# Kyaw-Thiha/animal-vision

Hardware: AMD Instinct MI355X
Metric: megapixels/sec per-frame pipeline (higher is better)
Workload: dtype f16

## Files before the change

### animal-vision_amd/csrc/mst_fused.hip

```cpp
#include <hip/hip_fp16.h>

#include <cstdio>
#include <cstdlib>
#include <cstring>

#include "avx_internal.h"
#include "mst_common.h"
#include "mst_tile_order.h"

namespace {

typedef float float4_t __attribute__((ext_vector_type(4)));
#ifndef AVX_FFN32_GM2
#define AVX_FFN32_GM2 1
#endif
constexpr int kFT = 512;
constexpr int TS = 16;
constexpr int HS = TS + 2;
#ifndef AVX_FFN_TH
#define AVX_FFN_TH 16
#endif
constexpr int kFfnTH = AVX_FFN_TH;
static_assert(kFfnTH == 14 || kFfnTH == 16, "FeedForward tile rows");
constexpr int kFfnNGRP = (HS * (kFfnTH + 2) + 31) / 32;
// ... 753 lines not shown
        uint2 xr[STASH ? 1 : NOUT];
        const int yo0 = t.y0 + 2 * rpo + (q >> 1), xo = t.x0 + n16;
        const bool livex = n16 < TW && xo < W;
        const size_t e0 = ((t.b * H + (yo0 < H ? yo0 : 0)) * (size_t)W + (livex ? xo : 0)) * C + 8 * oc + 4 * (q & 1), estep = (size_t)2 * W * C;
        auto live = [&](int u) { return livex && yo0 + 2 * u < H; };
        if constexpr (!STASH) {
#pragma unroll
            for (int u = 0; u < NOUT; ++u) xr[u] = live(u) ? *reinterpret_cast<const uint2*>(x + e0 + u * estep) : uint2{0, 0};
        }
        {
            const bool mid_inside = t.y0 >= 1 && t.y0 + MR - 1 <= H && t.x0 >= 1 && t.x0 + 15 <= W;
            uint4 bq[3];
            auto rd = [&](int u) {
#pragma unroll
                for (int i = 0; i < 3; ++i) bq[i] = *reinterpret_cast<const uint4*>(rbB + (size_t)(2 * (rpo + u)) * RP + i * PP + ob);
            };
            auto finish = [&](int u, float4_t a) {
                float2_t gp[2] = {float2_t{a[0], a[1]}, float2_t{a[2], a[3]}};
                if constexpr (C >= 64) gelu_mx<2>(gp);
                else { float2_t g0[1] = {gp[0]}, g1[1] = {gp[1]}; gelu_mx<1>(g0); gelu_mx<1>(g1); gp[0] = g0[0]; gp[1] = g1[0]; }
                uint2 ov = uint2{pack_f16(gp[0].x, gp[0].y), pack_f16(gp[1].x, gp[1].y)};
                if (!mid_inside) {
                    const int yy = t.y0 - 1 + 2 * (rpo + u) + (q >> 1), xx = t.x0 - 1 + n16;
                    const unsigned keep = (yy >= 0 && yy < H && xx >= 0 && xx < W) ? 0xffffffffu : 0u;
                    ov.x &= keep; ov.y &= keep;
                }
                *reinterpret_cast<uint2*>(wbB + (size_t)(2 * (rpo + u)) * MP + ob) = ov;
            };
            rd(0);
            float4_t prev = {0.f, 0.f, 0.f, 0.f};
#pragma unroll
            for (int u = 0; u < NMID; ++u) {
                float4_t acc = {0.f, 0.f, 0.f, 0.f};
#pragma unroll
                for (int i = 0; i < 3; ++i) acc = __builtin_amdgcn_mfma_f32_16x16x32_f16(a1[i], __builtin_bit_cast(half8_t, bq[i]), acc, 0, 0, 0);
                if (u + 1 < NMID) rd(u + 1);
                __builtin_amdgcn_sched_barrier(0);
                if (u > 0) finish(u - 1, prev);
                __builtin_amdgcn_sched_barrier(0);
                prev = acc;
            }
            finish(NMID - 1, prev);
        }
        stamp(2);
        {
            uint4 bq[3], bg[NK];
            uint2 xn = uint2{0, 0};
            const unsigned char* rbX = xs + (size_t)((q >> 1) * TW + n16) * PP + 16 * o + 8 * (q & 1);
            auto rd = [&](int u) {
#pragma unroll
                for (int i = 0; i < 3; ++i) bq[i] = *reinterpret_cast<const uint4*>(rbC + (size_t)(2 * (rpo + u)) * MP + i * PP + ob);
#pragma unroll
                for (int t2 = 0; t2 < NK; ++t2) bg[t2] = *reinterpret_cast<const uint4*>(rbG + (size_t)(2 * (rpo + u)) * RP + 32 * t2);
                if constexpr (STASH) xn = *reinterpret_cast<const uint2*>(rbX + (size_t)(2 * (rpo + u)) * TW * PP);
            };
            auto finish = [&](int u, float4_t acc, uint2 xu) {
                if (live(u)) {
                    constexpr unsigned kOnes = 0x3c003c00u;
                    float s0 = acc[0] + bs[0], s1 = acc[1] + bs[1], s2 = acc[2] + bs[2], s3 = acc[3] + bs[3];
                    fma_mix_lo(s0, xu.x, kOnes); fma_mix_hi(s1, xu.x, kOnes);
                    fma_mix_lo(s2, xu.y, kOnes); fma_mix_hi(s3, xu.y, kOnes);
                    *reinterpret_cast<uint2*>(out + e0 + u * estep) = uint2{pack_f16(s0, s1), pack_f16(s2, s3)};
                }
            };
            rd(0);
#ifndef AVX_TAIL_PIPE2
#define AVX_TAIL_PIPE2 1
#endif
            if constexpr (STASH && (AVX_TAIL_PIPE2 == 2 || (AVX_TAIL_PIPE2 == 1 && C == 64))) {
                float4_t prev = {0.f, 0.f, 0.f, 0.f};
                uint2 xp = uint2{0, 0};
#pragma unroll
                for (int u = 0; u < NOUT; ++u) {
                    const uint2 xu = xn;
                    float4_t acc = {0.f, 0.f, 0.f, 0.f};
#pragma unroll
                    for (int i = 0; i < 3; ++i) acc = __builtin_amdgcn_mfma_f32_16x16x32_f16(a2[i], __builtin_bit_cast(half8_t, bq[i]), acc, 0, 0, 0);
#pragma unroll
                    for (int t2 = 0; t2 < NK; ++t2) acc = __builtin_amdgcn_mfma_f32_16x16x32_f16(am[t2], __builtin_bit_cast(half8_t, bg[t2]), acc, 0, 0, 0);
                    if (u + 1 < NOUT) rd(u + 1);
                    __builtin_amdgcn_sched_barrier(0);
                    if (u > 0) finish(u - 1, prev, xp);
                    __builtin_amdgcn_sched_barrier(0);
                    prev = acc; xp = xu;
                }
                finish(NOUT - 1, prev, xp);
            } else {
#pragma unroll
                for (int u = 0; u < NOUT; ++u) {
                    const uint2 xu = STASH ? xn : xr[STASH ? 0 : u];
                    float4_t acc = {0.f, 0.f, 0.f, 0.f};
#pragma unroll
                    for (int i = 0; i < 3; ++i) acc = __builtin_amdgcn_mfma_f32_16x16x32_f16(a2[i], __builtin_bit_cast(half8_t, bq[i]), acc, 0, 0, 0);
#pragma unroll
                    for (int t2 = 0; t2 < NK; ++t2) acc = __builtin_amdgcn_mfma_f32_16x16x32_f16(am[t2], __builtin_bit_cast(half8_t, bg[t2]), acc, 0, 0, 0);
                    if (u + 1 < NOUT) rd(u + 1);
                    finish(u, acc, xu);
                }
            }
        }
        }
        stamp(3);
        if (!ahead.live) break;
        t = tile_at(ahead, TW, TR);
        ahead.advance();
        __syncthreads();
        stamp(4);
    }
    if constexpr (STAMP) {
        if (lane == 0 && stamps)
#pragma unroll
            for (int kk = 0; kk < 8; ++kk) stamps[((size_t)blockIdx.x * NW + wave) * 8 + kk] = seg[kk];
    }
}

template <int C, int TR, int MINW, int NW = 8>
int launch_attn_tail_mx(avx_ctx* ctx, const void* x, const void* wvpack, const void* mpack, const void* dw1, const void* dw2, const float* bias, void* out, int B, int H, int W,
                        hipStream_t s) {
    constexpr int PP = C * 2 + 16, RP = (18 * PP + 255) / 256 * 256;
    const size_t lds = (size_t)(TR + 4) * RP + (size_t)(TR + 2) * 16 * PP + (size_t)(C / 32) * (C / 16) * 1024 + ((C <= 64 && NW == 8) ? (size_t)(TR * 14 + 2) * PP : 0) ;
    const long total = (long)B * ((H + TR - 1) / TR) * ((W + 13) / 14);
    const long cap = (long)ctx->num_cus * (NW == 16 ? 1 : MINW / 2);
    AVX_REQUIRE(ctx, total <= 0x7fffffffl, "avx_mst_attn_tail_mx: 2^31 tiles or more");
    const unsigned blocks = (unsigned)(total < cap ? total : cap);
    if (getenv("AVX_TAIL_STAMPS")) {
        auto ks = k_mst_attn_tail_mx<C, TR, MINW, true, NW>;
        unsigned long long* d_st = nullptr;
        const size_t n = (size_t)blocks * NW * 8;
        AVX_HIP(ctx, hipMalloc((void**)&d_st, n * sizeof(unsigned long long)));
        AVX_HIP(ctx, hipFuncSetAttribute((const void*)ks, hipFuncAttributeMaxDynamicSharedMemorySize, (int)lds));
        hipLaunchKernelGGL(ks, dim3(blocks), dim3(64 * NW), lds, s, (const __half*)x, (const uint4*)wvpack, (const uint4*)mpack, (const uint4*)dw1, (const uint4*)dw2, bias, (__half*)out, B, H, W, d_st, mst_tile_order());
        AVX_HIP(ctx, hipStreamSynchronize(s));
        unsigned long long* h_st = (unsigned long long*)malloc(n * sizeof(unsigned long long));
        AVX_HIP(ctx, hipMemcpy(h_st, d_st, n * sizeof(unsigned long long), hipMemcpyDeviceToHost));
        double tot[8] = {0}, all = 0;
        for (size_t i = 0; i < n; ++i) { tot[i & 7] += (double)h_st[i]; all += (double)h_st[i]; }
        const char* nm[8] = {"v from x", "bar1", "conv1+gelu", "conv2+proj+store", "bar2", "-", "-", "-"};
        fprintf(stderr, "[tail stamps C=%d] %u blocks, %ld tiles, mean cycles per wave %.0f:", C, blocks, total, all / (blocks * (double)NW));
        for (int k2 = 0; k2 < 8; ++k2) fprintf(stderr, "  %s %.1f%%", nm[k2], 100 * tot[k2] / all);
        fprintf(stderr, "\n");
        free(h_st);
        (void)hipFree(d_st);
        return AVX_OK;
    }
    auto k = k_mst_attn_tail_mx<C, TR, MINW, false, NW>;
    AVX_HIP(ctx, hipFuncSetAttribute((const void*)k, hipFuncAttributeMaxDynamicSharedMemorySize, (int)lds));
    hipLaunchKernelGGL(k, dim3(blocks), dim3(64 * NW), lds, s, (const __half*)x, (const uint4*)wvpack, (const uint4*)mpack, (const uint4*)dw1,
                       (const uint4*)dw2, bias, (__half*)out, B, H, W, (unsigned long long*)nullptr, mst_tile_order());
    AVX_HIP(ctx, hipGetLastError());
    return AVX_OK;
}


struct SpecStat3 { float mn, mx; double sum; };
template <int MINW, bool GRAM, bool SPEC = false>
__global__ __launch_bounds__(kFT, MINW) void k_mst_conv3x3_lds(const __half* __restrict__ x , const uint4* __restrict__ wpack ,
                                                               const __half* __restrict__ add , __half* __restrict__ out, int B, int H, int W,
                                                               const uint4* __restrict__ wqk , float* __restrict__ partial ,
                                                               const float* __restrict__ specw = nullptr ,
                                                               float* __restrict__ planes = nullptr , SpecStat3* __restrict__ spart = nullptr ,
                                                               int crop_t = 0, int crop_l = 0, int Hc = 0, int Wc = 0, int order = AVX_TILE_ORDER_RASTER ) {
    constexpr int C = 32, PP = C * 2 + 16, RP = (HS * PP + 255) / 256 * 256, NFILL = (HS * HS * 4 + kFT - 1) / kFT;
    __shared__ __align__(16) unsigned char xt[HS * RP];
    __shared__ uint4 wl[18 * 64];
    const int tid = threadIdx.x, lane = tid & 63, wave = tid >> 6, p = lane & 31, h = lane >> 5;
    for (int i = tid; i < 18 * 64; i += kFT) wl[i] = wpack[i];
    __shared__ uint4 wq[GRAM ? 4 * 64 : 1];
    float16_t G;
    float nq = 0.f, nk = 0.f;
    if constexpr (GRAM) {
        if (tid < 4 * 64) wq[tid] = wqk[tid];
#pragma unroll
        for (int v = 0; v < 16; ++v) G[v] = 0.f;
    }
    float smn[3] = {3.4e38f, 3.4e38f, 3.4e38f}, smx[3] = {-3.4e38f, -3.4e38f, -3.4e38f};
    double ssum[3] = {0.0, 0.0, 0.0};
    const int tx = (W + TS - 1) / TS, ty = (H + TS - 1) / TS;
    uint4 pre[NFILL];
    unsigned f_rel[NFILL];
#pragma unroll
    for (int k = 0; k < NFILL; ++k) {
        const int it = tid + k * kFT, itc = it < HS * HS * 4 ? it : 0, q = itc >> 2, part = itc & 3;
        f_rel[k] = (unsigned)(((q / HS) * W + q % HS) * C + 8 * part) * 2u;
    }
    auto fetch = [&](const Tile& t) {
        if (t.y0 >= 1 && t.y0 + HS - 1 <= H && t.x0 >= 1 && t.x0 + HS - 1 <= W) {
            const char* origin = reinterpret_cast<const char*>(x + ((t.b * H + t.y0 - 1) * (size_t)W + t.x0 - 1) * C);
#pragma unroll
            for (int k = 0; k < NFILL; ++k) {
                unsigned o = f_rel[k];
                asm volatile("" : "+v"(o));
                pre[k] = *reinterpret_cast<const uint4*>(origin + o);
            }
            return;
        }
#pragma unroll
        for (int k = 0; k < NFILL; ++k) {
            const int it = tid + k * kFT, q = it >> 2, part = it & 3;
            const int yy = t.y0 - 1 + q / HS, xx = t.x0 - 1 + q % HS;
            const bool ok = it < HS * HS * 4 && yy >= 0 && yy < H && xx >= 0 && xx < W;
            const int yc = yy < 0 ? 0 : (yy >= H ? H - 1 : yy), xc = xx < 0 ? 0 : (xx >= W ? W - 1 : xx);
            uint4 r = *reinterpret_cast<const uint4*>(x + ((t.b * H + yc) * (size_t)W + xc) * C + 8 * part);
            r.x = ok ? r.x : 0u; r.y = ok ? r.y : 0u; r.z = ok ? r.z : 0u; r.w = ok ? r.w : 0u;
            pre[k] = r;
        }
    };
    TileWalk ahead;
    ahead.init(blockIdx.x, gridDim.x, B, ty, tx, (GRAM || SPEC) ? (int)AVX_TILE_ORDER_RASTER : order);
    if (!ahead.live) return;
    Tile t = tile_at(ahead, TS, TS);
    ahead.advance();
    fetch(t);
    for (;;) {
#pragma unroll
        for (int k = 0; k < NFILL; ++k) {
            const int it = tid + k * kFT, q = it >> 2, part = it & 3;
            if (it < HS * HS * 4) *reinterpret_cast<uint4*>(xt + (size_t)(q / HS) * RP + (size_t)(q % HS) * PP + 16 * part) = pre[k];
        }
        __syncthreads();
        if (ahead.live) fetch(tile_at(ahead, TS, TS));
        {
            const int r = 2 * wave + (p >> 4), c = p & 15;
            const int yo = t.y0 + r, xo = t.x0 + c;
            const bool live = yo < H && xo < W;
            const size_t off = ((t.b * H + (live ? yo : 0)) * (size_t)W + (live ? xo : 0)) * C + 16 * h;
            uint4 ar[2] = {uint4{0, 0, 0, 0}, uint4{0, 0, 0, 0}};
            if (add) { ar[0] = reinterpret_cast<const uint4*>(add + off)[0]; ar[1] = reinterpret_cast<const uint4*>(add + off)[1]; }
            float16_t d;
#pragma unroll
            for (int v = 0; v < 16; ++v) d[v] = 0.f;
            const unsigned char* src = xt + (size_t)r * RP + (size_t)c * PP + 16 * h;
#pragma unroll
            for (int tap = 0; tap < 9; ++tap)
#pragma unroll
                for (int s2 = 0; s2 < 2; ++s2)
                    d = mfma16(__builtin_bit_cast(half8_t, wl[(2 * tap + s2) * 64 + lane]), __builtin_bit_cast(half8_t, *reinterpret_cast<const uint4*>(src + (size_t)(tap / 3) * RP + (size_t)(tap % 3) * PP + 32 * s2)), d);
            half8_t o0, o1;
            {
                const half8_t r0 = __builtin_bit_cast(half8_t, ar[0]), r1 = __builtin_bit_cast(half8_t, ar[1]);
#pragma unroll
                for (int v = 0; v < 8; ++v) { o0[v] = (_Float16)(d[v] + (float)r0[v]); o1[v] = (_Float16)(d[8 + v] + (float)r1[v]); }
            }
            if constexpr (SPEC) {
                float a3[3] = {0.f, 0.f, 0.f};
                auto chain = [&]() {
#pragma unroll
                    for (int j = 0; j < 16; ++j) {
                        const float v = (float)(j < 8 ? o0[j] : o1[j - 8]);
                        const float* wb = specw + (16 * h + j) * 4;
#pragma unroll
                        for (int k = 0; k < 3; ++k) a3[k] = __builtin_fmaf(v, wb[k], a3[k]);
                    }
                };
                if (h == 0) chain();
#pragma unroll
                for (int k = 0; k < 3; ++k) { const float lo = __shfl_xor(a3[k], 32); a3[k] = h ? lo : a3[k]; }
                if (h == 1) chain();
                const int yc = yo - crop_t, xc = xo - crop_l;
                if (h == 1 && live && yc >= 0 && yc < Hc && xc >= 0 && xc < Wc) {
#pragma unroll
                    for (int k = 0; k < 3; ++k) {
                        planes[(size_t)k * Hc * Wc + (size_t)yc * Wc + xc] = a3[k];
                        smn[k] = fminf(smn[k], a3[k]); smx[k] = fmaxf(smx[k], a3[k]); ssum[k] += (double)a3[k];
                    }
                }
            } else if (live) {
                reinterpret_cast<uint4*>(out + off)[0] = __builtin_bit_cast(uint4, o0);
                reinterpret_cast<uint4*>(out + off)[1] = __builtin_bit_cast(uint4, o1);
            }
            if constexpr (GRAM) {
                if (!live) { o0 = half8_t{0, 0, 0, 0, 0, 0, 0, 0}; o1 = o0; }
                float16_t dq, dk;
#pragma unroll
                for (int v = 0; v < 16; ++v) { dq[v] = 0.f; dk[v] = 0.f; }
                dq = mfma16(o0, __builtin_bit_cast(half8_t, wq[0 * 64 + lane]), dq);
                dq = mfma16(o1, __builtin_bit_cast(half8_t, wq[1 * 64 + lane]), dq);
                dk = mfma16(o0, __builtin_bit_cast(half8_t, wq[2 * 64 + lane]), dk);
                dk = mfma16(o1, __builtin_bit_cast(half8_t, wq[3 * 64 + lane]), dk);
                unsigned aq[8], ak[8];
#pragma unroll
                for (int j = 0; j < 8; ++j) {
                    aq[j] = pack_f16(dq[2 * j], dq[2 * j + 1]);
                    ak[j] = pack_f16(dk[2 * j], dk[2 * j + 1]);
                    fma_mix_lo(nq, aq[j], aq[j]); fma_mix_hi(nq, aq[j], aq[j]);
                    fma_mix_lo(nk, ak[j], ak[j]); fma_mix_hi(nk, ak[j], ak[j]);
                }
#pragma unroll
                for (int b2 = 0; b2 < 2; ++b2)
                    G = mfma16(__builtin_bit_cast(half8_t, uint4{ak[4 * b2], ak[4 * b2 + 1], ak[4 * b2 + 2], ak[4 * b2 + 3]}),
                               __builtin_bit_cast(half8_t, uint4{aq[4 * b2], aq[4 * b2 + 1], aq[4 * b2 + 2], aq[4 * b2 + 3]}), G);
            }
        }
        if (!ahead.live) break;
        t = tile_at(ahead, TS, TS);
        ahead.advance();
        __syncthreads();
    }
    if constexpr (SPEC) {
        __syncthreads();
        float* redf = reinterpret_cast<float*>(xt);
        double* redd = reinterpret_cast<double*>(xt + 256);
#pragma unroll
        for (int k = 0; k < 3; ++k) {
            float a = smn[k], b2 = smx[k];
            double c2 = ssum[k];
#pragma unroll
            for (int o = 32; o > 0; o >>= 1) { a = fminf(a, __shfl_xor(a, o)); b2 = fmaxf(b2, __shfl_xor(b2, o)); c2 += __shfl_xor(c2, o); }
            if (lane == 0) { redf[(wave * 3 + k) * 2] = a; redf[(wave * 3 + k) * 2 + 1] = b2; redd[wave * 3 + k] = c2; }
        }
        __syncthreads();
        if (tid < 3) {
            float a = 3.4e38f, b2 = -3.4e38f;
            double c2 = 0.0;
            for (int w8 = 0; w8 < 8; ++w8) { a = fminf(a, redf[(w8 * 3 + tid) * 2]); b2 = fmaxf(b2, redf[(w8 * 3 + tid) * 2 + 1]); c2 += redd[w8 * 3 + tid]; }
            spart[(size_t)blockIdx.x * 3 + tid] = SpecStat3{a, b2, c2};
        }
    }
    if constexpr (GRAM) {
        static_assert(sizeof(xt) >= sizeof(float) * 4 * 34 * 32, "the halo tile's LDS holds four waves' results at a time");
        float* red = reinterpret_cast<float*>(xt);
        const float sq = nq + __shfl_xor(nq, 32), sk = nk + __shfl_xor(nk, 32);
        float sum[3] = {0.f, 0.f, 0.f};
#pragma unroll
        for (int half = 0; half < 2; ++half) {
            __syncthreads();
            if ((wave >> 2) == half) {
                float* mine = red + (size_t)(wave & 3) * 34 * 32;
#pragma unroll
                for (int v = 0; v < 16; ++v) mine[(8 * (v / 4) + 4 * h + (v % 4)) * 32 + p] = G[v];
                if (h == 0) { mine[32 * 32 + p] = sq; mine[33 * 32 + p] = sk; }
            }
            __syncthreads();
#pragma unroll
            for (int q = 0; q < 3; ++q) {
                const int i = tid + q * kFT;
                if (i < 34 * 32)
#pragma unroll
                    for (int w4 = 0; w4 < 4; ++w4) sum[q] += red[(size_t)w4 * 34 * 32 + i];
            }
        }
#pragma unroll
        for (int q = 0; q < 3; ++q) {
            const int i = tid + q * kFT;
            if (i < 34 * 32) partial[(size_t)blockIdx.x * 34 * 32 + i] = sum[q];
        }
    }
}


template <int C>
struct DownGeo {
    static constexpr int OH = C == 32 ? 8 : 4, OW = 16, IH = 2 * OH + 2, IW = 2 * OW + 2;
    static constexpr int NP = C / 8;
    static constexpr int RPS = IW * NP + (C == 32 ? 2 : 4);
    static constexpr int NI = ((IH * RPS + 63) / 64 + 7) / 8 * 8;
    static constexpr int PER_WAVE = NI / 8, BUF = NI * 1024, NBUF = C == 32 ? 3 : 2, GROUPS = OH / 2;
    static constexpr int PART = C == 32 ? 0 : 2 * 4 * 4096;
    __device__ static int swz(int col) { return C == 32 ? (col >> 2) & 3 : (col >> 1) & 7; }
};
#pragma clang diagnostic push
#pragma clang diagnostic ignored "-Winline-asm"
__device__ __forceinline__ void lds_dma16(const void* g, unsigned lds_base ) {
    asm volatile("s_mov_b32 m0, %0\n\ts_nop 0\n\tglobal_load_lds_dwordx4 %1, off" ::"s"(__builtin_amdgcn_readfirstlane(lds_base)), "v"(g) : "memory", "m0");
}
__device__ __forceinline__ void lds_dma16(const void* base , unsigned ofs, unsigned lds_base) {
    asm volatile("s_mov_b32 m0, %0\n\ts_nop 0\n\tglobal_load_lds_dwordx4 %1, %2" ::"s"(__builtin_amdgcn_readfirstlane(lds_base)), "v"(ofs), "s"(base) : "memory", "m0");
}
#pragma clang diagnostic pop
template <int C>
__global__ __launch_bounds__(kFT, 2) void k_mst_down4x4_dma(const __half* __restrict__ x , const uint4* __restrict__ wpack ,
                                                            __half* __restrict__ out , const void* __restrict__ zero, int B, int H, int W, int order ) {
    using G = DownGeo<C>;
    constexpr int CO = 2 * C, NT = CO / 32, KS = C / 16;
    __shared__ __align__(1024) unsigned char lds[G::NBUF * G::BUF + G::PART];
    const int tid = threadIdx.x, lane = tid & 63, wave = __builtin_amdgcn_readfirstlane(tid >> 6) , p = lane & 31, h = lane >> 5;
    const int g0 = C == 32 ? wave & 3 : 0, nt = C == 32 ? wave >> 2 : wave & 3, kh = C == 32 ? 0 : wave >> 2;
    half8_t wf[32];
#pragma unroll
    for (int i = 0; i < 32; ++i) {
        const int tap = C == 32 ? i >> 1 : 8 * kh + (i >> 2), s2 = C == 32 ? i & 1 : i & 3;
        wf[i] = __builtin_bit_cast(half8_t, wpack[((size_t)(tap * NT + nt) * KS + s2) * 64 + lane]);
    }
    const int Ho = H / 2, Wo = W / 2;
    const int tx = (Wo + G::OW - 1) / G::OW, ty = (Ho + G::OH - 1) / G::OH;
    struct T2 { int ox0, oy0, b; };
    auto tile_at = [&](const TileWalk& w) { return T2{w.xi * G::OW, w.yi * G::OH, w.b}; };
    int rel[G::PER_WAVE], rc[G::PER_WAVE];
#pragma unroll
    for (int k = 0; k < G::PER_WAVE; ++k) {
        const int L = (wave + 8 * k) * 64 + lane, row = L / G::RPS, rem = L - row * G::RPS, col = rem / G::NP, j = (rem - col * G::NP) ^ G::swz(col);
        const bool inside = row < G::IH && col < G::IW;
        rel[k] = inside ? (row * W + col) * (C * 2) + 16 * j : 0;
        rc[k] = inside ? row << 8 | col : -1;
    }
    const unsigned lds0 = __builtin_amdgcn_readfirstlane((unsigned)(size_t)(__attribute__((address_space(3))) unsigned char*)lds);
    auto fill = [&](const TileWalk& w, int slot) {
        const bool exists = w.live;
        const T2 t = tile_at(w);
        const int y0 = 2 * t.oy0 - 1, x0 = 2 * t.ox0 - 1;
        const char* origin = reinterpret_cast<const char*>(x) + (((long)t.b * H + y0) * W + x0) * (long)(C * 2);
        const unsigned lb = lds0 + slot * G::BUF + wave * 1024;
        if (exists && y0 >= 0 && y0 + G::IH <= H && x0 >= 0 && x0 + G::IW <= W) {
#pragma unroll
            for (int k = 0; k < G::PER_WAVE; ++k) lds_dma16(origin , (unsigned)rel[k], lb + k * 8192);
        } else {
#pragma unroll
            for (int k = 0; k < G::PER_WAVE; ++k) {
                const int yy = y0 + (rc[k] >> 8), xx = x0 + (rc[k] & 255);
                const bool ok = exists && rc[k] >= 0 && yy >= 0 && yy < H && xx >= 0 && xx < W;
                lds_dma16(ok ? (const void*)(origin + rel[k]) : zero, lb + k * 8192);
            }
        }
    };
    TileWalk walk, look;
    walk.init(blockIdx.x, gridDim.x, B, ty, tx, order);
    if (!walk.live) return;
    look = walk;
#pragma unroll
    for (int a = 0; a < G::NBUF - 1; ++a) { fill(look, a); look.advance(); }
    const int c2 = 2 * (p & 15);
    int colofs[4];
#pragma unroll
    for (int kx = 0; kx < 4; ++kx) colofs[kx] = (c2 + kx) * G::NP;
    int slot = 0, plain_stores = 0;
    for (;;) {
        if (plain_stores == G::NBUF - 1 && (C == 32 || kh == 0)) asm volatile("s_waitcnt vmcnt(%0)" ::"n"(G::PER_WAVE * (G::NBUF - 2) + 2 * (C == 32 ? 1 : G::GROUPS) * (G::NBUF - 1)) : "memory");
        else asm volatile("s_waitcnt vmcnt(%0)" ::"n"(G::PER_WAVE * (G::NBUF - 2)) : "memory");
        __syncthreads();
        {
            int nslot = slot + G::NBUF - 1;
            nslot -= nslot >= G::NBUF ? G::NBUF : 0;
            fill(look, nslot);
            look.advance();
        }
        const T2 t = tile_at(walk);
        const bool whole = t.oy0 + G::OH <= Ho && t.ox0 + G::OW <= Wo;
        const unsigned char* bt = lds + slot * G::BUF;
#pragma unroll 1
        for (int g = g0; g < (C == 32 ? g0 + 1 : G::GROUPS); ++g) {
            const int r = 2 * g + (p >> 4);
            float16_t d, d1;
#pragma unroll
            for (int v = 0; v < 16; ++v) d[v] = 0.f, d1[v] = 0.f;
            const unsigned char* src = bt + (size_t)(2 * r) * (G::RPS * 16);
            auto frag = [&](int i) {
                const int tap = C == 32 ? i >> 1 : 8 * kh + (i >> 2), s2 = C == 32 ? i & 1 : i & 3, ky = tap >> 2, kx = tap & 3;
                return *reinterpret_cast<const uint4*>(src + ky * (G::RPS * 16) + (colofs[kx] + ((2 * s2 + h) ^ G::swz(c2 + kx))) * 16);
            };
            constexpr int AHEAD = 6;
            uint4 bq[AHEAD];
#pragma unroll
// ... 161 lines not shown
            if (visit && k < steps_cap) visit[(size_t)wg * steps_cap + k] = ((long long)wk.b * ty + wk.yi) * tx + wk.xi;
        if (visit)
            for (int r = k; r < steps_cap; ++r) visit[(size_t)wg * steps_cap + r] = -1;
        most = k > most ? k : most;
    }
    if (steps_out) *steps_out = most;
    return AVX_OK;
}

extern "C" int avx_mst_ffn_fused(avx_ctx* ctx, const void* x, const float* gamma, const float* beta, float eps, const void* w1pack, const void* taps_9xhid,
                                 const void* w2pack, void* out, int B, int H, int W, int C, void* stream) {
    if (!ctx) return AVX_ERR_INVALID;
    AVX_REQUIRE(ctx, taps_9xhid, "avx_mst_ffn_fused: NULL pointer");
    return ffn_fused_launch(ctx, x, gamma, beta, eps, w1pack, taps_9xhid, nullptr, w2pack, out, B, H, W, C, stream);
}

extern "C" int avx_mst_ffn_fused_mx(avx_ctx* ctx, const void* x, const float* gamma, const float* beta, float eps, const void* w1pack, const void* dwpack,
                                    const void* w2pack, void* out, int B, int H, int W, int C, void* stream) {
    if (!ctx) return AVX_ERR_INVALID;
    AVX_REQUIRE(ctx, dwpack && (((uintptr_t)dwpack) & 15u) == 0, "avx_mst_ffn_fused_mx: dwpack NULL or not 16-byte aligned");
    return ffn_fused_launch(ctx, x, gamma, beta, eps, w1pack, nullptr, dwpack, w2pack, out, B, H, W, C, stream);
}

static int ffn_fused_launch(avx_ctx* ctx, const void* x, const float* gamma, const float* beta, float eps, const void* w1pack, const void* taps_9xhid, const void* dwpack,
                            const void* w2pack, void* out, int B, int H, int W, int C, void* stream) {
    AVX_REQUIRE(ctx, x && gamma && beta && w1pack && w2pack && out && B > 0 && H > 0 && W > 0, "avx_mst_ffn_fused: NULL pointer or empty tensor");
    AVX_REQUIRE(ctx, C == 32 || C == 64 || C == 128, "avx_mst_ffn_fused: C=%d (32, 64 or 128: 31-channel groups stored 32 wide)", C);
    AVX_REQUIRE(ctx, ((((uintptr_t)x | (uintptr_t)w1pack | (uintptr_t)w2pack | (uintptr_t)out | (uintptr_t)taps_9xhid)) & 15u) == 0,
                "avx_mst_ffn_fused: pointers must be 16-byte aligned");
    AVX_REQUIRE(ctx, x != out, "avx_mst_ffn_fused: neighbouring tiles read each other's halo: the output cannot be the input");
    AVX_HIP(ctx, hipSetDevice(ctx->device));
    hipStream_t s = avx_pick_stream(ctx, stream);
    const long total = (long)B * ((H + kFfnTH - 1) / kFfnTH) * ((W + TS - 1) / TS);
    const char* hp = getenv("AVX_MST_FFN_HPASS");
    const bool small = C == 32 && !(hp && atoi(hp) == 128);
    const int hpass = (small || C == 128) ? 64 : 128, hpitch = hpass * 2 + 16, rpitch = (HS * hpitch + 255) / 256 * 256;
    const long cap = (long)ctx->num_cus * (small ? 2 : 1);
    const bool nw16 = C == 64 && dwpack && !(getenv("AVX_MST_FFN_NW") && atoi(getenv("AVX_MST_FFN_NW")) == 8);
    const size_t lds = (size_t)kFfnNGRP * 32 * (C * 2 + 16) + (size_t)(kFfnTH + 2) * rpitch + (dwpack ? 0 : (size_t)9 * 4 * C * 2) + sizeof(float) * 2 * C + (nw16 ? (size_t)(C / 32) * (hpass / 16) * 1024 : 0);
    AVX_REQUIRE(ctx, total <= 0x7fffffffl, "avx_mst_ffn_fused: 2^31 tiles or more");
    const dim3 grid((unsigned)(total < cap ? total : cap));
    const int order = mst_tile_order();
#define AVX_FFN1(CV, HP, MW, DW, NWV)                                                                                                            \
    {                                                                                                                                            \
        auto k = k_mst_ffn_fused<CV, HP, MW, DW, false, NWV>;                                                                                    \
        AVX_HIP(ctx, hipFuncSetAttribute((const void*)k, hipFuncAttributeMaxDynamicSharedMemorySize, (int)lds));                                 \
        hipLaunchKernelGGL(k, grid, dim3(64 * NWV), lds, s, (const __half*)x, gamma, beta, eps, (const uint4*)w1pack, (const __half*)taps_9xhid, \
                           (const uint4*)w2pack, (__half*)out, B, H, W, (const uint4*)dwpack, (unsigned long long*)nullptr, order);              \
    }
#define AVX_FFN(CV, HP, MW) { if (dwpack) AVX_FFN1(CV, HP, MW, true, 8) else AVX_FFN1(CV, HP, MW, false, 8) }
    if (dwpack && getenv("AVX_FFN_STAMPS") && ((C == 32 && small) || C == 64 || C == 128)) {
        unsigned long long* d_st = nullptr;
        const int nwv = nw16 ? 16 : 8;
        const size_t n = (size_t)grid.x * nwv * 8;
        AVX_HIP(ctx, hipMalloc((void**)&d_st, n * sizeof(unsigned long long)));
#define AVX_FFN_ST(CV, HP, MW, NWV)                                                                                                              \
    {                                                                                                                                            \
        auto k = k_mst_ffn_fused<CV, HP, MW, true, true, NWV>;                                                                                   \
        AVX_HIP(ctx, hipFuncSetAttribute((const void*)k, hipFuncAttributeMaxDynamicSharedMemorySize, (int)lds));                                 \
        hipLaunchKernelGGL(k, grid, dim3(64 * NWV), lds, s, (const __half*)x, gamma, beta, eps, (const uint4*)w1pack, (const __half*)taps_9xhid, \
                           (const uint4*)w2pack, (__half*)out, B, H, W, (const uint4*)dwpack, d_st, order);                                      \
    }
        if (C == 32) AVX_FFN_ST(32, 64, 4, 8) else if (nw16) AVX_FFN_ST(64, 128, 1, 16) else if (C == 64) AVX_FFN_ST(64, 128, 2, 8) else AVX_FFN_ST(128, 64, 2, 8)
#undef AVX_FFN_ST
        AVX_HIP(ctx, hipStreamSynchronize(s));
        unsigned long long* h_st = (unsigned long long*)malloc(n * sizeof(unsigned long long));
        AVX_HIP(ctx, hipMemcpy(h_st, d_st, n * sizeof(unsigned long long), hipMemcpyDeviceToHost));
        double tot[8] = {0}, w0[8] = {0}, w7[8] = {0};
        for (size_t i = 0; i < n; ++i) { tot[i & 7] += (double)h_st[i]; if (((i >> 3) % nwv) == 0) w0[i & 7] += (double)h_st[i]; if (((i >> 3) % nwv) == (size_t)nwv - 1) w7[i & 7] += (double)h_st[i]; }
        double all = 0;
        for (int k2 = 0; k2 < 8; ++k2) all += tot[k2];
        fprintf(stderr, "[ffn stamps C=%d] %u blocks x %d waves, mean cycles per wave %.0f; share per segment (all waves | first wave | last wave): ", C, grid.x, nwv, all / (grid.x * (double)nwv));
        const char* nm[8] = {"bar1", "phase1", "bar2", "phase2a", "bar3", "phase2b", "epilogue", "ln+fetch"};
        for (int k2 = 0; k2 < 8; ++k2) fprintf(stderr, "%s %.1f%% | %.1f%% | %.1f%%  ", nm[k2], 100 * tot[k2] / all, 100 * w0[k2] * nwv / all, 100 * w7[k2] * nwv / all);
        fprintf(stderr, "\n");
        free(h_st);
        (void)hipFree(d_st);
    } else if (C == 32 && small) AVX_FFN(32, 64, 4) else if (C == 32) AVX_FFN(32, 128, 2)
    else if (nw16) AVX_FFN1(64, 128, 1, true, 16)
    else if (C == 64) AVX_FFN(64, 128, 2) else AVX_FFN(128, 64, 2)
#undef AVX_FFN
#undef AVX_FFN1
    AVX_HIP(ctx, hipGetLastError());
    return AVX_OK;
}

extern "C" int avx_mst_attn_tail(avx_ctx* ctx, const void* v, const void* x, const void* mpack16, const void* taps1_9xc, const void* taps2_9xc, const float* bias,
                                 void* out, int B, int H, int W, int C, void* stream) {
    if (!ctx) return AVX_ERR_INVALID;
    AVX_REQUIRE(ctx, v && x && mpack16 && taps1_9xc && taps2_9xc && out && B > 0 && H > 0 && W > 0, "avx_mst_attn_tail: NULL pointer or empty tensor");
    AVX_REQUIRE(ctx, C == 32 || C == 64, "avx_mst_attn_tail: C=%d (32 or 64)", C);
    AVX_REQUIRE(ctx, ((((uintptr_t)v | (uintptr_t)x | (uintptr_t)mpack16 | (uintptr_t)out | (uintptr_t)taps1_9xc | (uintptr_t)taps2_9xc)) & 15u) == 0,
                "avx_mst_attn_tail: pointers must be 16-byte aligned");
    AVX_REQUIRE(ctx, v != out, "avx_mst_attn_tail: tiles read their neighbours' rows of v: the output cannot be v (it may be x)");
    AVX_HIP(ctx, hipSetDevice(ctx->device));
    hipStream_t s = avx_pick_stream(ctx, stream);
    if (C == 32) return launch_attn_tail<32, 4>(ctx, v, x, mpack16, taps1_9xc, taps2_9xc, bias, out, B, H, W, s, nullptr);
    return launch_attn_tail<64, 2>(ctx, v, x, mpack16, taps1_9xc, taps2_9xc, bias, out, B, H, W, s, nullptr);
}

extern "C" int avx_mst_attn_tail_x(avx_ctx* ctx, const void* x, const void* wvpack16, const void* mpack16, const void* taps1_9xc, const void* taps2_9xc,
                                   const float* bias, void* out, int B, int H, int W, int C, void* stream) {
    if (!ctx) return AVX_ERR_INVALID;
    AVX_REQUIRE(ctx, x && wvpack16 && mpack16 && taps1_9xc && taps2_9xc && out && B > 0 && H > 0 && W > 0, "avx_mst_attn_tail_x: NULL pointer or empty tensor");
    AVX_REQUIRE(ctx, C == 32 || C == 64, "avx_mst_attn_tail_x: C=%d (32 or 64)", C);
    AVX_REQUIRE(ctx, ((((uintptr_t)x | (uintptr_t)wvpack16 | (uintptr_t)mpack16 | (uintptr_t)out | (uintptr_t)taps1_9xc | (uintptr_t)taps2_9xc)) & 15u) == 0,
                "avx_mst_attn_tail_x: pointers must be 16-byte aligned");
    AVX_REQUIRE(ctx, x != out, "avx_mst_attn_tail_x: tiles read their neighbours' rows of x: the output cannot be x");
    AVX_HIP(ctx, hipSetDevice(ctx->device));
    hipStream_t s = avx_pick_stream(ctx, stream);
    if (C == 32) return launch_attn_tail<32, 4>(ctx, x, x, mpack16, taps1_9xc, taps2_9xc, bias, out, B, H, W, s, wvpack16);
    return launch_attn_tail<64, 2>(ctx, x, x, mpack16, taps1_9xc, taps2_9xc, bias, out, B, H, W, s, wvpack16);
}

extern "C" int avx_mst_attn_tail_mx(avx_ctx* ctx, const void* x, const void* wvpack16, const void* mpack_mx, const void* dw1pack, const void* dw2pack,
                                    const float* bias, void* out, int B, int H, int W, int C, void* stream) {
    if (!ctx) return AVX_ERR_INVALID;
    AVX_REQUIRE(ctx, x && wvpack16 && mpack_mx && dw1pack && dw2pack && out && B > 0 && H > 0 && W > 0, "avx_mst_attn_tail_mx: NULL pointer or empty tensor");
    AVX_REQUIRE(ctx, C == 32 || C == 64 || C == 128, "avx_mst_attn_tail_mx: C=%d (32, 64 or 128)", C);
    AVX_REQUIRE(ctx, ((((uintptr_t)x | (uintptr_t)wvpack16 | (uintptr_t)mpack_mx | (uintptr_t)out | (uintptr_t)dw1pack | (uintptr_t)dw2pack)) & 15u) == 0,
                "avx_mst_attn_tail_mx: pointers must be 16-byte aligned");
    AVX_REQUIRE(ctx, x != out, "avx_mst_attn_tail_mx: tiles read their neighbours' rows of x: the output cannot be x");
    AVX_HIP(ctx, hipSetDevice(ctx->device));
    hipStream_t s = avx_pick_stream(ctx, stream);
    if (C == 32) return launch_attn_tail_mx<32, 16, 4>(ctx, x, wvpack16, mpack_mx, dw1pack, dw2pack, bias, out, B, H, W, s);
    if (C == 128) return launch_attn_tail_mx<128, 8, 2>(ctx, x, wvpack16, mpack_mx, dw1pack, dw2pack, bias, out, B, H, W, s);
    if (getenv("AVX_MST_TAIL_NW") && atoi(getenv("AVX_MST_TAIL_NW")) == 16) return launch_attn_tail_mx<64, 16, 1, 16>(ctx, x, wvpack16, mpack_mx, dw1pack, dw2pack, bias, out, B, H, W, s);
    return launch_attn_tail_mx<64, 16, 2>(ctx, x, wvpack16, mpack_mx, dw1pack, dw2pack, bias, out, B, H, W, s);
}

extern "C" int avx_mst_conv3x3_lds(avx_ctx* ctx, const void* x, const void* wpack16, const void* add, void* out, int B, int H, int W, int C, void* stream) {
    if (!ctx) return AVX_ERR_INVALID;
    AVX_REQUIRE(ctx, x && wpack16 && out && B > 0 && H > 0 && W > 0, "avx_mst_conv3x3_lds: NULL pointer or empty tensor");
    AVX_REQUIRE(ctx, C == 32, "avx_mst_conv3x3_lds: C=%d (32: the 31-channel full-resolution convs)", C);
    AVX_REQUIRE(ctx, ((((uintptr_t)x | (uintptr_t)wpack16 | (uintptr_t)add | (uintptr_t)out)) & 15u) == 0, "avx_mst_conv3x3_lds: pointers must be 16-byte aligned");
    AVX_REQUIRE(ctx, x != out, "avx_mst_conv3x3_lds: in-place convolution is not possible");
    AVX_HIP(ctx, hipSetDevice(ctx->device));
    hipStream_t s = avx_pick_stream(ctx, stream);
    const long total = (long)B * ((H + TS - 1) / TS) * ((W + TS - 1) / TS);
    const long cap = (long)ctx->num_cus * 3;
    AVX_REQUIRE(ctx, total <= 0x7fffffffl, "avx_mst_conv3x3_lds: 2^31 tiles or more");
    hipLaunchKernelGGL((k_mst_conv3x3_lds<6, false>), dim3((unsigned)(total < cap ? total : cap)), dim3(kFT), 0, s, (const __half*)x, (const uint4*)wpack16, (const __half*)add,
                       (__half*)out, B, H, W, (const uint4*)nullptr, (float*)nullptr, (const float*)nullptr, (float*)nullptr, (SpecStat3*)nullptr, 0, 0, 0, 0, mst_tile_order());
    AVX_HIP(ctx, hipGetLastError());
    return AVX_OK;
}

extern "C" int avx_mst_conv3x3_lds_spectral(avx_ctx* ctx, const void* x, const void* wpack16, const void* add, int H, int W, int C, const float* weights_host, int crop_t,
                                            int crop_l, int Hc, int Wc, float* planes_out, void* partials_out, int* n_partials, void* stream) {
    if (!ctx) return AVX_ERR_INVALID;
    AVX_REQUIRE(ctx, x && wpack16 && weights_host && planes_out && partials_out && n_partials && H > 0 && W > 0, "avx_mst_conv3x3_lds_spectral: NULL pointer or empty tensor");
    AVX_REQUIRE(ctx, C == 32, "avx_mst_conv3x3_lds_spectral: C=%d (32: the 31-band cube as stored)", C);
    AVX_REQUIRE(ctx, crop_t >= 0 && crop_l >= 0 && Hc > 0 && Wc > 0 && crop_t + Hc <= H && crop_l + Wc <= W, "avx_mst_conv3x3_lds_spectral: the crop window must lie inside the frame");
    AVX_REQUIRE(ctx, ((((uintptr_t)x | (uintptr_t)wpack16 | (uintptr_t)add | (uintptr_t)partials_out)) & 15u) == 0, "avx_mst_conv3x3_lds_spectral: pointers must be 16-byte aligned");
    AVX_HIP(ctx, hipSetDevice(ctx->device));
    hipStream_t s = avx_pick_stream(ctx, stream);
    avx_ws* ws = avx_workspace(ctx, s);
    if (!ws) return AVX_ERR_NOMEM;
    float wT[32 * 4];
    for (int b = 0; b < 32; ++b)
        for (int k = 0; k < 4; ++k) wT[b * 4 + k] = k < 3 ? weights_host[(size_t)k * 32 + b] : 0.0f;
    float* dwT = nullptr;
    int rc = avx_const_upload(ctx, ws, 2, wT, sizeof(wT), s, (void**)&dwT);
    if (rc) return rc;
    const long total = (long)((H + TS - 1) / TS) * ((W + TS - 1) / TS);
    const long cap = (long)ctx->num_cus * 2;
    const long blocks = total < cap ? total : cap;
    *n_partials = (int)blocks;
    hipLaunchKernelGGL((k_mst_conv3x3_lds<4, false, true>), dim3((unsigned)blocks), dim3(kFT), 0, s, (const __half*)x, (const uint4*)wpack16, (const __half*)add, (__half*)nullptr, 1, H, W,
                       (const uint4*)nullptr, (float*)nullptr, (const float*)dwT, planes_out, (SpecStat3*)partials_out, crop_t, crop_l, Hc, Wc);
    AVX_HIP(ctx, hipGetLastError());
    return AVX_OK;
}

extern "C" int avx_mst_conv3x3_lds_gram(avx_ctx* ctx, const void* x, const void* wpack16, const void* add, void* out, int H, int W, int C, const void* wqk16, float* gram,
                                        float* nq, float* nk, void* stream) {
    if (!ctx) return AVX_ERR_INVALID;
    AVX_REQUIRE(ctx, x && wpack16 && out && wqk16 && gram && nq && nk && H > 0 && W > 0, "avx_mst_conv3x3_lds_gram: NULL pointer or empty tensor");
    AVX_REQUIRE(ctx, C == 32, "avx_mst_conv3x3_lds_gram: C=%d (32: the 31-channel full-resolution convs)", C);
    AVX_REQUIRE(ctx, ((((uintptr_t)x | (uintptr_t)wpack16 | (uintptr_t)add | (uintptr_t)out | (uintptr_t)wqk16)) & 15u) == 0, "avx_mst_conv3x3_lds_gram: pointers must be 16-byte aligned");
    AVX_REQUIRE(ctx, x != out, "avx_mst_conv3x3_lds_gram: in-place convolution is not possible");
    AVX_HIP(ctx, hipSetDevice(ctx->device));
    hipStream_t s = avx_pick_stream(ctx, stream);
    avx_ws* ws = avx_workspace(ctx, s);
    if (!ws) return AVX_ERR_NOMEM;
    const long total = (long)((H + TS - 1) / TS) * ((W + TS - 1) / TS);
    const long cap = (long)ctx->num_cus * 2;
    const long blocks = total < cap ? total : cap;
    int rc = avx_ensure_scratch(ctx, ws, sizeof(float) * (size_t)blocks * 34 * 32);
    if (rc) return rc;
    float* partial = (float*)ws->d_scratch;
    hipLaunchKernelGGL((k_mst_conv3x3_lds<4, true>), dim3((unsigned)blocks), dim3(kFT), 0, s, (const __half*)x, (const uint4*)wpack16, (const __half*)add, (__half*)out, 1, H, W,
                       (const uint4*)wqk16, partial);
    AVX_HIP(ctx, hipGetLastError());
    return avx_mst_qkv_final_launch(ctx, partial, (int)blocks, 1, gram, nq, nk, s);
}

extern "C" int avx_mst_conv_in_u8(avx_ctx* ctx, const uint8_t* frame_hwc, int H, int W, int pad_top, int pad_bottom, int pad_left, int pad_right,
                                  const float* w_27x32_dev, void* out, void* stream) {
    if (!ctx) return AVX_ERR_INVALID;
    AVX_REQUIRE(ctx, frame_hwc && w_27x32_dev && out && H > 1 && W > 1, "avx_mst_conv_in_u8: NULL pointer or a frame too small to reflect");
    AVX_REQUIRE(ctx, pad_top >= 0 && pad_bottom >= 0 && pad_left >= 0 && pad_right >= 0 && pad_top < H && pad_bottom < H && pad_left < W && pad_right < W,
                "avx_mst_conv_in_u8: reflect padding must be smaller than the frame");
    AVX_REQUIRE(ctx, ((uintptr_t)out & 15u) == 0, "avx_mst_conv_in_u8: out must be 16-byte aligned");
    AVX_HIP(ctx, hipSetDevice(ctx->device));
    hipStream_t s = avx_pick_stream(ctx, stream);
    const int Hp = H + pad_top + pad_bottom, Wp = W + pad_left + pad_right;
    const size_t total = (size_t)Hp * Wp;
    const size_t want = (total + 255) / 256, cap = (size_t)ctx->num_cus * 16;
    if (getenv("AVX_MST_CONV_IN_VALU"))
        hipLaunchKernelGGL(k_mst_conv_in_u8, dim3((unsigned)(want < cap ? want : cap)), dim3(256), 0, s, frame_hwc, w_27x32_dev, (__half*)out, H, W, pad_top, pad_left, Hp, Wp);
    else {
        const size_t wantm = (total + 127) / 128;
        hipLaunchKernelGGL(k_mst_conv_in_u8_mfma, dim3((unsigned)(wantm < cap ? wantm : cap)), dim3(256), 0, s, frame_hwc, w_27x32_dev, (__half*)out, H, W, pad_top,
                           pad_left, Hp, Wp);
    }
    AVX_HIP(ctx, hipGetLastError());
    return AVX_OK;
}

extern "C" int avx_mst_down4x4(avx_ctx* ctx, const void* x, const void* wpack16, void* out, int B, int H, int W, int C, void* stream) {
    if (!ctx) return AVX_ERR_INVALID;
    AVX_REQUIRE(ctx, x && wpack16 && out && B > 0 && H > 0 && W > 0, "avx_mst_down4x4: NULL pointer or empty tensor");
    AVX_REQUIRE(ctx, C == 32 || C == 64, "avx_mst_down4x4: C=%d (32 or 64: the encoder steps 31 -> 62 and 62 -> 124 channels as stored)", C);
    AVX_REQUIRE(ctx, H % 2 == 0 && W % 2 == 0, "avx_mst_down4x4: H and W must be even (the model pads frames to multiples of 8)");
    AVX_REQUIRE(ctx, (long)B * H * W * C * 2 < (1l << 31), "avx_mst_down4x4: input larger than 2 GiB");
    AVX_REQUIRE(ctx, ((((uintptr_t)x | (uintptr_t)wpack16 | (uintptr_t)out)) & 15u) == 0, "avx_mst_down4x4: pointers must be 16-byte aligned");
    AVX_HIP(ctx, hipSetDevice(ctx->device));
    hipStream_t s = avx_pick_stream(ctx, stream);
    const long cap = (long)ctx->num_cus;
    if (C == 32) {
        using G = DownGeo<32>;
        const long total = (long)B * ((H / 2 + G::OH - 1) / G::OH) * ((W / 2 + G::OW - 1) / G::OW);
        hipLaunchKernelGGL(k_mst_down4x4_dma<32>, dim3((unsigned)(total < cap ? total : cap)), dim3(kFT), 0, s, (const __half*)x, (const uint4*)wpack16, (__half*)out, (const void*)ctx->d_zero, B, H, W, mst_tile_order());
    } else {
        using G = DownGeo<64>;
        const long total = (long)B * ((H / 2 + G::OH - 1) / G::OH) * ((W / 2 + G::OW - 1) / G::OW);
        hipLaunchKernelGGL(k_mst_down4x4_dma<64>, dim3((unsigned)(total < cap ? total : cap)), dim3(kFT), 0, s, (const __half*)x, (const uint4*)wpack16, (__half*)out, (const void*)ctx->d_zero, B, H, W, mst_tile_order());
    }
    AVX_HIP(ctx, hipGetLastError());
    return AVX_OK;
}
```

Measured before the change: 429.4.

## Software-pipeline spectral epilogue across tiles and stage spectral weights in LDS

The spectral projection epilogue of the fused conv3x3 kernel is restructured. The old version ran the two half-wave chains one after the other, with a shuffle between them inside each tile. Now the second half-wave processes the previous tile's values while the first half processes the current tile, with carried registers and a final drain pass after the loop. The 32x4 spectral weights are also staged into LDS instead of being read from global memory per FMA. This removes serialized idle half-waves, at the cost of extra live registers and a tail pass. A 32-bit pixel-index guard is added.

Result: no change. 431.7, median of 5 (+0.5%).

```diff
diff --git a/animal-vision_amd/csrc/mst_fused.hip b/animal-vision_amd/csrc/mst_fused.hip
--- a/animal-vision_amd/csrc/mst_fused.hip
+++ b/animal-vision_amd/csrc/mst_fused.hip
@@ -929,6 +929,12 @@
 }
 
 
+#ifndef AVX_SPEC_EPI_LDSW
+#define AVX_SPEC_EPI_LDSW 1
+#endif
+#ifndef AVX_SPEC_EPI_PIPE
+#define AVX_SPEC_EPI_PIPE 1
+#endif
 struct SpecStat3 { float mn, mx; double sum; };
 template <int MINW, bool GRAM, bool SPEC = false>
 __global__ __launch_bounds__(kFT, MINW) void k_mst_conv3x3_lds(const __half* __restrict__ x , const uint4* __restrict__ wpack ,
@@ -942,6 +948,14 @@
     __shared__ uint4 wl[18 * 64];
     const int tid = threadIdx.x, lane = tid & 63, wave = tid >> 6, p = lane & 31, h = lane >> 5;
     for (int i = tid; i < 18 * 64; i += kFT) wl[i] = wpack[i];
+    __shared__ float4 sw[SPEC && AVX_SPEC_EPI_LDSW ? 32 : 1];
+    if constexpr (SPEC && AVX_SPEC_EPI_LDSW) {
+        if (tid < 32 * 4) reinterpret_cast<float*>(sw)[tid] = specw[tid];
+    }
+    constexpr unsigned kSpecDead = 0xffffffffu;
+    half8_t pv0 = half8_t{0, 0, 0, 0, 0, 0, 0, 0}, pv1 = pv0;
+    float hand[3] = {0.f, 0.f, 0.f};
+    unsigned pidx = kSpecDead;
     __shared__ uint4 wq[GRAM ? 4 * 64 : 1];
     float16_t G;
     float nq = 0.f, nk = 0.f;
@@ -981,6 +995,39 @@
             r.x = ok ? r.x : 0u; r.y = ok ? r.y : 0u; r.z = ok ? r.z : 0u; r.w = ok ? r.w : 0u;
             pre[k] = r;
         }
+    };
+    auto spec_chain = [&](float (&a3)[3], const half8_t b0, const half8_t b1) {
+#pragma unroll
+        for (int j = 0; j < 16; ++j) {
+            float w3[3];
+            if constexpr (AVX_SPEC_EPI_LDSW) {
+                const float4 wb = sw[16 * h + j];
+                w3[0] = wb.x; w3[1] = wb.y; w3[2] = wb.z;
+            } else {
+                const float* wb = specw + (16 * h + j) * 4;
+#pragma unroll
+                for (int k = 0; k < 3; ++k) w3[k] = wb[k];
+            }
+            const float v = (float)(j < 8 ? b0[j] : b1[j - 8]);
+#pragma unroll
+            for (int k = 0; k < 3; ++k) a3[k] = __builtin_fmaf(v, w3[k], a3[k]);
+        }
+    };
+    auto spec_put = [&](const float (&a3)[3], const size_t at) {
+#pragma unroll
+        for (int k = 0; k < 3; ++k) {
+            planes[(size_t)k * Hc * Wc + at] = a3[k];
+            smn[k] = fminf(smn[k], a3[k]); smx[k] = fmaxf(smx[k], a3[k]); ssum[k] += (double)a3[k];
+        }
+    };
+    auto spec_pass = [&](const half8_t b0, const half8_t b1) {
+        float a3[3];
+#pragma unroll
+        for (int k = 0; k < 3; ++k) a3[k] = h ? hand[k] : 0.f;
+        spec_chain(a3, b0, b1);
+        if (h == 1 && pidx != kSpecDead) spec_put(a3, pidx);
+#pragma unroll
+        for (int k = 0; k < 3; ++k) hand[k] = __shfl_xor(a3[k], 32);
     };
     TileWalk ahead;
     ahead.init(blockIdx.x, gridDim.x, B, ty, tx, (GRAM || SPEC) ? (int)AVX_TILE_ORDER_RASTER : order);
@@ -1019,26 +1066,33 @@
                 for (int v = 0; v < 8; ++v) { o0[v] = (_Float16)(d[v] + (float)r0[v]); o1[v] = (_Float16)(d[8 + v] + (float)r1[v]); }
             }
             if constexpr (SPEC) {
-                float a3[3] = {0.f, 0.f, 0.f};
-                auto chain = [&]() {
-#pragma unroll
-                    for (int j = 0; j < 16; ++j) {
-                        const float v = (float)(j < 8 ? o0[j] : o1[j - 8]);
-                        const float* wb = specw + (16 * h + j) * 4;
-#pragma unroll
-                        for (int k = 0; k < 3; ++k) a3[k] = __builtin_fmaf(v, wb[k], a3[k]);
-                    }
-                };
-                if (h == 0) chain();
-#pragma unroll
-                for (int k = 0; k < 3; ++k) { const float lo = __shfl_xor(a3[k], 32); a3[k] = h ? lo : a3[k]; }
-                if (h == 1) chain();
                 const int yc = yo - crop_t, xc = xo - crop_l;
-                if (h == 1 && live && yc >= 0 && yc < Hc && xc >= 0 && xc < Wc) {
-#pragma unroll
-                    for (int k = 0; k < 3; ++k) {
-                        planes[(size_t)k * Hc * Wc + (size_t)yc * Wc + xc] = a3[k];
-                        smn[k] = fminf(smn[k], a3[k]); smx[k] = fmaxf(smx[k], a3[k]); ssum[k] += (double)a3[k];
+                if constexpr (AVX_SPEC_EPI_PIPE) {
+                    const bool keep = live && yc >= 0 && yc < Hc && xc >= 0 && xc < Wc;
+                    spec_pass(h ? pv0 : o0, h ? pv1 : o1);
+                    pv0 = o0; pv1 = o1;
+                    pidx = keep ? (unsigned)yc * (unsigned)Wc + (unsigned)xc : kSpecDead;
+                } else {
+                    float a3[3] = {0.f, 0.f, 0.f};
+                    auto chain = [&]() {
+#pragma unroll
+                        for (int j = 0; j < 16; ++j) {
+                            const float v = (float)(j < 8 ? o0[j] : o1[j - 8]);
+                            const float* wb = (AVX_SPEC_EPI_LDSW ? reinterpret_cast<const float*>(sw) : specw) + (16 * h + j) * 4;
+#pragma unroll
+                            for (int k = 0; k < 3; ++k) a3[k] = __builtin_fmaf(v, wb[k], a3[k]);
+                        }
+                    };
+                    if (h == 0) chain();
+#pragma unroll
+                    for (int k = 0; k < 3; ++k) { const float lo = __shfl_xor(a3[k], 32); a3[k] = h ? lo : a3[k]; }
+                    if (h == 1) chain();
+                    if (h == 1 && live && yc >= 0 && yc < Hc && xc >= 0 && xc < Wc) {
+#pragma unroll
+                        for (int k = 0; k < 3; ++k) {
+                            planes[(size_t)k * Hc * Wc + (size_t)yc * Wc + xc] = a3[k];
+                            smn[k] = fminf(smn[k], a3[k]); smx[k] = fmaxf(smx[k], a3[k]); ssum[k] += (double)a3[k];
+                        }
                     }
                 }
             } else if (live) {
@@ -1074,6 +1128,7 @@
         __syncthreads();
     }
     if constexpr (SPEC) {
+        if constexpr (AVX_SPEC_EPI_PIPE) spec_pass(pv0, pv1);
         __syncthreads();
         float* redf = reinterpret_cast<float*>(xt);
         double* redd = reinterpret_cast<double*>(xt + 256);
@@ -1541,6 +1596,7 @@
     AVX_REQUIRE(ctx, x && wpack16 && weights_host && planes_out && partials_out && n_partials && H > 0 && W > 0, "avx_mst_conv3x3_lds_spectral: NULL pointer or empty tensor");
     AVX_REQUIRE(ctx, C == 32, "avx_mst_conv3x3_lds_spectral: C=%d (32: the 31-band cube as stored)", C);
     AVX_REQUIRE(ctx, crop_t >= 0 && crop_l >= 0 && Hc > 0 && Wc > 0 && crop_t + Hc <= H && crop_l + Wc <= W, "avx_mst_conv3x3_lds_spectral: the crop window must lie inside the frame");
+    AVX_REQUIRE(ctx, (long)Hc * Wc < 0xffffffffl, "avx_mst_conv3x3_lds_spectral: 2^32 - 1 pixels or more in a plane");
     AVX_REQUIRE(ctx, ((((uintptr_t)x | (uintptr_t)wpack16 | (uintptr_t)add | (uintptr_t)partials_out)) & 15u) == 0, "avx_mst_conv3x3_lds_spectral: pointers must be 16-byte aligned");
     AVX_HIP(ctx, hipSetDevice(ctx->device));
     hipStream_t s = avx_pick_stream(ctx, stream);
```
